# mateomarin/two_towers

Measured on AMD Instinct MI355X. Metric: training pairs/sec at global batch=8192, 1/2/4/8 GPUs; MRR@10 match, higher is better.
Workload: dtype bf16; 1 GPU; BASELINE configs[2]: EnhancedTwoTowerModel(300, 256), seq_len 64, batch 8192 per GPU, bf16, hard-negative mining k=5 + margin 0.2, dropout 0.1, Adam; global_batch=8192, seq_len=64, hidden=256, embedding_dim=300, parallelism=dp1, loss=hardneg_margin

## Files before the change

two_towers_amd/csrc/tt_api.h:

```cpp
#pragma once
#include <hip/hip_runtime.h>
#include <stdio.h>
#include <string.h>

#include "../../include/tt_hip.h"

namespace tt {
void set_error(const char* fmt, ...);

enum Opt {
  OPT_GRU_STEP,
  OPT_GRU_DEPTH,
  OPT_GRU_BWD_ROWS,
  OPT_GRU_BWD_BIG,
  OPT_GRU_BWD_STREAMS,
  OPT_GEMM_PERSIST,
  OPT_GEMM_A3,
  OPT_GEMM_REGSTAGE,
  OPT_GEMM_STREAM_OUT,
  OPT_HN_GEMM,
  OPT_GRU_BWD_PERSIST,
  OPT_GRU_FWD_STEP_ROWS,
  OPT_INFONCE_FLASH,
  OPT_HN_MAP,
  OPT_GEMM_SKEW,
  OPT_GEMM_PERSIST_MAXK,
  OPT_GRU_FWD_XC,
  OPT_GRU_XC_SKIP,
  OPT_GRU_XC_SPINS,
  OPT_GRU_BWD_SKEW,
  OPT_GRU_FWD_SKEW,
  OPT_GEMM_BRES,
  OPT_GRU_XC_COOP,
  OPT_GEMM_BUF,
  OPT_GEMM_ORDER,
  OPT_GRU_STEP_RING,
  OPT_GRU_FWD_XS,
  OPT_HN_SCAN_GEMM,
  OPT_GEMM_IEPI,
  OPT_BRES_ROWS,
  OPT_HN_SCAN_V,
  OPT_GEMM_W4,
  OPT_N
};
int opt(Opt o);
int tt_hn_scan_gemm(const void* q, long bq, const void* d, long nd, int h, long label_off, float* cm, long nch,
                    hipStream_t st);
}

#define TT_CHECK_ARG(cond, ...)            \
  do {                                     \
    if (!(cond)) {                         \
      tt::set_error(__VA_ARGS__);          \
      return TT_EINVAL;                    \
    }                                      \
  } while (0)

#define TT_CHECK_LAUNCH(what)                                                        \
  do {                                                                               \
    hipError_t e_ = hipGetLastError();                                               \
    if (e_ != hipSuccess) {                                                          \
      tt::set_error("%s: %s", what, hipGetErrorString(e_));                          \
      return (int)e_;                                                                \
    }                                                                                \
  } while (0)

#define TT_CHECK_HIP(expr)                                                           \
  do {                                                                               \
    hipError_t e_ = (expr);                                                          \
    if (e_ != hipSuccess) {                                                          \
      tt::set_error("%s: %s", #expr, hipGetErrorString(e_));                         \
      return (int)e_;                                                                \
    }                                                                                \
  } while (0)

#define TT_PROPAGATE(expr)     \
  do {                         \
    int rc_ = (expr);          \
    if (rc_ != 0) return rc_;  \
  } while (0)

static inline int tt_ceil_div(long a, long b) { return (int)((a + b - 1) / b); }
```

two_towers_amd/csrc/tt_gemm.hip:

```cpp
#include <float.h>
#include <stdarg.h>
#include <stdlib.h>

#include <atomic>
#include <type_traits>

#include "tt_api.h"
#include "tt_gemm_core.h"

namespace tt {
static thread_local char g_err[512];
void set_error(const char* fmt, ...) {
  va_list ap;
  va_start(ap, fmt);
  vsnprintf(g_err, sizeof(g_err), fmt, ap);
  va_end(ap);
}
}

namespace tt {
namespace {
struct OptDef {
  const char* name;
  const char* env;
  int dflt;
};
constexpr OptDef kOpts[OPT_N] = {
    {"gru_step", "TT_GRU_STEP", 0},               {"gru_depth", "TT_GRU_DEPTH", 4},
    {"gru_bwd_rows", "TT_GRU_BWD_ROWS", 0},     {"gru_bwd_big", "TT_GRU_BWD_BIG", 1},
    {"gru_bwd_streams", "TT_GRU_BWD_STREAMS", 2}, {"gemm_persist", "TT_GEMM_PERSIST", 1},
    {"gemm_a3", "TT_GEMM_A3", 1},                 {"gemm_regstage", "TT_GEMM_REGSTAGE", 0},
    {"gemm_stream_out", "TT_GEMM_STREAM_OUT", 1}, {"hn_gemm", "TT_HN_GEMM", 0},
    {"gru_bwd_persist", "TT_GRU_BWD_PERSIST", 1}, {"gru_fwd_step_rows", "TT_GRU_FWD_STEP_ROWS", 0},
    {"infonce_flash", "TT_INFONCE_FLASH", 1},     {"hn_map", "TT_HN_MAP", 2},
    {"gemm_skew", "TT_GEMM_SKEW", 0},             {"gemm_persist_maxk", "TT_GEMM_PERSIST_MAXK", 24},
    {"gru_fwd_xc", "TT_GRU_FWD_XC", 1},           {"gru_xc_skip", "TT_GRU_XC_SKIP", 0},
    {"gru_xc_spins", "TT_GRU_XC_SPINS", 22},      {"gru_bwd_skew", "TT_GRU_BWD_SKEW", 14},
    {"gru_fwd_skew", "TT_GRU_FWD_SKEW", 0},       {"gemm_bres", "TT_GEMM_BRES", 1},
    {"gru_xc_coop", "TT_GRU_XC_COOP", 0},         {"gemm_buf", "TT_GEMM_BUF", 1},
    {"gemm_order", "TT_GEMM_ORDER", 0},           {"gru_step_ring", "TT_GRU_STEP_RING", 4},
    {"gru_fwd_xs", "TT_GRU_FWD_XS", 1},           {"hn_scan_gemm", "TT_HN_SCAN_GEMM", 0},
    {"gemm_iepi", "TT_GEMM_IEPI", 1},             {"bres_rows", "TT_BRES_ROWS", 32},
    {"hn_scan_v", "TT_HN_SCAN_V", 5},             {"gemm_w4", "TT_GEMM_W4", 0},
};
struct OptTable {
  std::atomic<int> v[OPT_N];
  OptTable() {
    for (int i = 0; i < OPT_N; ++i) {
      const char* e = getenv(kOpts[i].env);
      v[i].store(e && *e ? atoi(e) : kOpts[i].dflt, std::memory_order_relaxed);
    }
  }
};
OptTable& opts() {
  static OptTable t;
  return t;
}
int find_opt(const char* name) {
  for (int i = 0; name && i < OPT_N; ++i)
    if (strcmp(name, kOpts[i].name) == 0) return i;
  return -1;
}
}
int opt(Opt o) { return opts().v[o].load(std::memory_order_relaxed); }
}

extern "C" const char* tt_version(void) { return "tt_hip 0.2.0 gfx950"; }
extern "C" const char* tt_last_error(void) { return tt::g_err; }
extern "C" int tt_set_option(const char* name, int value) {
  const int i = tt::find_opt(name);
  TT_CHECK_ARG(i >= 0, "tt_set_option: unknown option '%s'", name ? name : "(null)");
  tt::opts().v[i].store(value, std::memory_order_relaxed);
  return 0;
}
extern "C" int tt_get_option(const char* name, int* value) {
  const int i = tt::find_opt(name);
  TT_CHECK_ARG(i >= 0 && value, "tt_get_option: unknown option '%s'", name ? name : "(null)");
  *value = tt::opt((tt::Opt)i);
  return 0;
}

namespace {

struct GemmArgs {
  const void* a[4];
  const void* b[4];
  void* c[4];
  const float* bias[4];
  int bshift[4];
  const void* a_hi[4];
  int a_split;
  long lda, ldb, ldc;
  int M, N, K;
  int splits, kt_per_split;
  float alpha;
  int beta, relu, seq_t;
  uint32_t drop_seed, drop_thresh, drop_row0;
  float drop_inv_keep;
  long part_stride;
  int vec_ok;
  int force_regstage;
  int skew;
  int bias_vec_ok;
  int stream_out;
  int walk_g, walk_x;
  int nbatch;
  float* cm;
  long nch, label_off;
};

constexpr int BM = 128, BN = 128;

#ifndef TT_TAIL_SKIP
#define TT_TAIL_SKIP 1
#endif
using ttg::xcd_remap;
#ifndef PERSIST_IEPI
#define PERSIST_IEPI 1
#endif
#ifndef PERSIST_BAL
#define PERSIST_BAL 1
#endif
#ifndef TT_EPI_PAIR
#define TT_EPI_PAIR 1
#endif
#ifndef TT_GEMM_BAL
// ... 1383 lines not shown
```

two_towers_amd/csrc/tt_gru.hip:

```cpp
#include <algorithm>
#include <cstdlib>
#include <mutex>
#include <type_traits>

#include "tt_api.h"
#include "tt_gemm_core.h"

namespace {

struct FwdRec {
  const void* g; const void* whh; const float* bhn; void* y; void* x1; void* save; float* hs;
  int dir; uint32_t seed; int col0;
  uint32_t row0;
};
struct FwdArgs {
  FwdRec r[4];
  int B, T, H;
  long ldg, ldy;
  int s;
  uint32_t drop_thresh;
  float inv_keep;
#ifdef TT_DIAG
  int dbg;
#endif
// ... 242 lines not shown
        if (!last) ld8(cr_nxt + (long)b * H + j, cin);
        else if (R.dfinal) ld8(R.dfinal + (long)b * a.ldf + j, cin);
        else {
#pragma unroll
          for (int e = 0; e < 8; ++e) cin[e] = 0.f;
        }
        if (DY) ld8(DY + row * a.ldy + j, dy);
        else {
#pragma unroll
          for (int e = 0; e < 8; ++e) dy[e] = 0.f;
        }
        const T* sp = S + row * S4 + j;
        ld8(sp, ar);
        ld8(sp + H, az);
        ld8(sp + 2 * H, an);
        ld8(sp + 3 * H, gh);
        if (s > 0) ld8(Y + ((long)b * T_ + tp) * a.ldy + j, hp);
        else {
#pragma unroll
          for (int e = 0; e < 8; ++e) hp[e] = 0.f;
        }
        const float* Lc = L + rl * BLD + jg;
        float o_r[8], o_z[8], o_n[8], o_hn[8], cout[8];
#pragma unroll
        for (int e = 0; e < 8; ++e) {
          const float dht = Lc[e] + cin[e] + dy[e];
          float rg, omr, zg, omz, ng, sech2;
          tt_sigmoid_pair(ar[e], rg, omr);
          tt_sigmoid_pair(az[e], zg, omz);
          tt_tanh_sech2(an[e], ng, sech2);
          const float dnp = dht * omz * sech2;
          const float drp = dnp * gh[e] * rg * omr;
          const float dzp = dht * (hp[e] - ng) * zg * omz;
          o_r[e] = drp; o_z[e] = dzp; o_n[e] = dnp; o_hn[e] = dnp * rg;
          cout[e] = dht * zg;
          bsum[0][e] += drp; bsum[1][e] += dzp; bsum[2][e] += dnp; bsum[3][e] += dnp * rg;
        }
        st8(cr_cur + (long)b * H + j, cout);
        T* xw = DGXw + row * a.ldd + j;
        st8(xw, o_r);
        st8(xw + H, o_z);
        const int go = (int)((((long)(b - m0) * T_) * a.ldd + j + 2 * H) * (long)sizeof(T));
        st8_sc1(grs, go, o_n, (T*)nullptr);
        st8(DGHw + row * a.ldd + j, o_hn);
      }
    }
    __syncthreads();
  }
#pragma unroll
  for (int q = 0; q < 4; ++q)
#pragma unroll
    for (int e = 0; e < 8; ++e) {
      float v = bsum[q][e];
      v += __shfl_xor(v, 16, 64);
      v += __shfl_xor(v, 32, 64);
      bsum[q][e] = v;
    }
  float* red = L;
  if (lane < 16) {
#pragma unroll
    for (int q = 0; q < 4; ++q)
#pragma unroll
      for (int e = 0; e < 8; ++e) red[(wave * 4 + q) * 128 + lane * 8 + e] = bsum[q][e];
  }
  __syncthreads();
  if (tid < 128 && j0 + tid < H) {
    float* pb = R.dbias + (long)mt * (4L * H) + j0 + tid;
#pragma unroll
    for (int q = 0; q < 4; ++q)
      pb[q * H] += red[(0 * 4 + q) * 128 + tid] + red[(1 * 4 + q) * 128 + tid] + red[(2 * 4 + q) * 128 + tid] +
                   red[(3 * 4 + q) * 128 + tid];
  }
}

TT_DEV void unpack8(uint4 v, float (&f)[8]) {
  f[0] = __uint_as_float(v.x << 16); f[1] = __uint_as_float(v.x & 0xFFFF0000u);
  f[2] = __uint_as_float(v.y << 16); f[3] = __uint_as_float(v.y & 0xFFFF0000u);
  f[4] = __uint_as_float(v.z << 16); f[5] = __uint_as_float(v.z & 0xFFFF0000u);
  f[6] = __uint_as_float(v.w << 16); f[7] = __uint_as_float(v.w & 0xFFFF0000u);
}

#ifndef TT_BWD_BUF
#define TT_BWD_BUF 1
#endif
#ifndef TT_BWD_STAG
#define TT_BWD_STAG 0
#endif
#ifndef TT_BWD_NB
#define TT_BWD_NB 2
#endif
#ifndef TT_BWD_NT
#define TT_BWD_NT 3
#endif
#ifndef TT_BWD_PIPE
#define TT_BWD_PIPE 1
#endif
#ifndef TT_BWD_CREG
#define TT_BWD_CREG 1
#endif
#ifndef TT_BWD_OUT_NT
#define TT_BWD_OUT_NT 0
#endif
template <bool NT>
TT_DEV void st8_pol(bf16_t* p, const float (&f)[8]) {
  if constexpr (NT) {
    tt_u32x4 w;
#pragma unroll
    for (int i = 0; i < 4; ++i) w[i] = (uint32_t)f2bf(f[2 * i]) | ((uint32_t)f2bf(f[2 * i + 1]) << 16);
    __builtin_nontemporal_store(w, reinterpret_cast<tt_u32x4*>(p));
  } else {
    st8(p, f);
  }
}

__global__ __launch_bounds__(512) void gru_bwd_big(BwdArgs a) {
  using L8 = ttg::Loop8<bf16_t, false, true, false, false, false, TT_BWD_BUF != 0>;
  static_assert(L8::LDS_BYTES >= 128 * 256 * 4 && L8::LDS_BYTES >= 8 * 4 * 256 * 4, "staging fits the slots");
  __shared__ __attribute__((aligned(16))) char lds[L8::LDS_BYTES];
  const int H = a.H, T_ = a.T, s = a.s;
  const int ntj = (H + 255) / 256, ntm = (a.B + 255) / 256;
  const int id = ttg::xcd_remap(blockIdx.x, gridDim.x);
  const int rz = id / (ntm * ntj), rem = id - rz * ntm * ntj;
  const int mt = rem / ntj;
  const BwdRec R = a.r[rz];
  const int m0 = mt * 256, j0 = (rem % ntj) * 256;
  const int t = R.dir ? T_ - 1 - s : s;
  const int tn = R.dir ? t - 1 : t + 1;
  const int tp = R.dir ? t + 1 : t - 1;
  const bool last = (s == T_ - 1);
  const int wave = threadIdx.x >> 6, lane = threadIdx.x & 63, tid = threadIdx.x;
  const int wn = (wave & 3) * 64;

  f32x4 acc[8][4];
#pragma unroll
  for (int i = 0; i < 8; ++i)
#pragma unroll
    for (int j = 0; j < 4; ++j) acc[i][j] = f32x4{0.f, 0.f, 0.f, 0.f};
#ifdef TT_DIAG
  const int dbg = a.dbg;
#else
  constexpr int dbg = 0;
#endif
  if (!last && !(dbg & 1)) {
    const bf16_t* DGX = static_cast<const bf16_t*>(R.dgx);
    const bf16_t* DGH = static_cast<const bf16_t*>(R.dgh);
    ttg::KCSplit<bf16_t> la{DGX + (long)tn * a.ldd, DGH + (long)tn * a.ldd, (long)T_ * a.ldd, m0, a.B, 2 * H};
    ttg::KOPlain<bf16_t> lb{static_cast<const bf16_t*>(R.whh), H, j0, H - j0};
    L8::run(la, lb, 3 * H, 0, (3 * H + L8::KTE - 1) / L8::KTE, lds, acc);
  }

  float* L = reinterpret_cast<float*>(lds);
  const int cur = s & 1, nxt = cur ^ 1;
  const bf16_t* S = static_cast<const bf16_t*>(R.save);
  const bf16_t* Y = static_cast<const bf16_t*>(R.y);
  const bf16_t* DY = static_cast<const bf16_t*>(R.dy);
  bf16_t* DGXw = static_cast<bf16_t*>(R.dgx);
  bf16_t* DGHw = static_cast<bf16_t*>(R.dgh);
  bf16_t* cr_cur = static_cast<bf16_t*>(R.dh) + (long)cur * a.B * H;
  const bf16_t* cr_nxt = static_cast<const bf16_t*>(R.dh) + (long)nxt * a.B * H;
  const long S4 = 4L * H;
  const int jg = (tid & 31) * 8;
  const int j = j0 + jg;
  const __amdgpu_buffer_rsrc_t grs = tt_rsrc(DGXw + ((long)m0 * T_ + t) * a.ldd);
  const __amdgpu_buffer_rsrc_t rc = tt_rsrc_n(cr_nxt + (long)m0 * H, !last);
  const __amdgpu_buffer_rsrc_t rd = tt_rsrc_n(DY ? DY + ((long)m0 * T_ + t) * a.ldy : S, DY != nullptr);
  const __amdgpu_buffer_rsrc_t rsv = tt_rsrc_n(S + ((long)m0 * T_ + t) * S4, true);
  const __amdgpu_buffer_rsrc_t ry = tt_rsrc_n(s > 0 ? Y + ((long)m0 * T_ + tp) * a.ldy : S, s > 0);
  float bsum[4][8];
#pragma unroll
// ... 17 lines not shown
#pragma unroll
      for (int kk = 0; kk < NB; ++kk) {
        const int bl = (tid >> 5) + p * 64 + 16 * ((kb + kk) & 3) + 128 * ((kb + kk) >> 2);
        const bool ok = m0 + bl < a.B && !(dbg & 2);
        const uint32_t oc = ok ? (uint32_t)(bl * H + j) * 2u : 0x80000000u;
        const uint32_t oy = ok ? (uint32_t)(bl * T_ * (int)a.ldy + j) * 2u : 0x80000000u;
        const uint32_t os = ok ? (uint32_t)(bl * T_ * (int)S4 + j) * 2u : 0x80000000u;
        vin[kk][0] = ld16_buf(rc, oc, 0);
        vin[kk][1] = ld16_buf<(TT_BWD_NT & 2) ? 2 : 0>(rd, oy, 0);
#pragma unroll
        for (int q = 0; q < 4; ++q) vin[kk][2 + q] = ld16_buf<(TT_BWD_NT & 1) ? 2 : 0>(rsv, os, q * 2 * H);
        vin[kk][6] = ld16_buf<(TT_BWD_NT & 2) ? 2 : 0>(ry, oy, 0);
      }
#pragma unroll
      for (int kk = 0; kk < NB; ++kk) {
        const int rl = (tid >> 5) + 16 * (kb + kk);
        const int b = m0 + (rl >> 6) * 128 + p * 64 + (rl & 63);
        if (b >= a.B) continue;
        const long row = (long)b * T_ + t;
        float cin[8], dy[8], ar[8], az[8], an[8], gh[8], hp[8];
        unpack8(vin[kk][0], cin);
        unpack8(vin[kk][1], dy);
        unpack8(vin[kk][2], ar);
        unpack8(vin[kk][3], az);
        unpack8(vin[kk][4], an);
        unpack8(vin[kk][5], gh);
        unpack8(vin[kk][6], hp);
        if (last && R.dfinal) ld8(R.dfinal + (long)b * a.ldf + j, cin);
        const float* Lc = L + rl * 256 + jg;
        float o_r[8], o_z[8], o_n[8], o_hn[8], cout[8];
#pragma unroll
        for (int e = 0; e < 8; ++e) {
          const float dht = Lc[e] + cin[e] + dy[e];
          float rg, omr, zg, omz, ng, sech2;
          tt_sigmoid_pair(ar[e], rg, omr);
          tt_sigmoid_pair(az[e], zg, omz);
          tt_tanh_sech2(an[e], ng, sech2);
          const float dnp = dht * omz * sech2;
          const float drp = dnp * gh[e] * rg * omr;
          const float dzp = dht * (hp[e] - ng) * zg * omz;
          o_r[e] = drp; o_z[e] = dzp; o_n[e] = dnp; o_hn[e] = dnp * rg;
          cout[e] = dht * zg;
          bsum[0][e] += drp; bsum[1][e] += dzp; bsum[2][e] += dnp; bsum[3][e] += dnp * rg;
        }
        if (dbg & 4) {
          if (o_r[0] == 12345.f) L[0] = o_z[1] + o_n[2] + o_hn[3] + cout[4];
          continue;
        }
        st8(cr_cur + (long)b * H + j, cout);
        bf16_t* xw = DGXw + row * a.ldd + j;
        st8(xw, o_r);
        st8(xw + H, o_z);
        const int go = (int)((((long)(b - m0) * T_) * a.ldd + j + 2 * H) * 2L);
        st8_sc1(grs, go, o_n, (bf16_t*)nullptr);
        st8(DGHw + row * a.ldd + j, o_hn);
      }
    }
    __syncthreads();
  }
#pragma unroll
  for (int q = 0; q < 4; ++q)
#pragma unroll
    for (int e = 0; e < 8; ++e) bsum[q][e] += __shfl_xor(bsum[q][e], 32, 64);
  float* red = L;
  if (lane < 32) {
#pragma unroll
    for (int q = 0; q < 4; ++q)
#pragma unroll
      for (int e = 0; e < 8; ++e) red[(wave * 4 + q) * 256 + lane * 8 + e] = bsum[q][e];
  }
  __syncthreads();
  if (tid < 256 && j0 + tid < H) {
    float* pb = R.dbias + (long)(mt * 2) * (4L * H) + j0 + tid;
#pragma unroll
    for (int q = 0; q < 4; ++q) {
      float v = 0.f;
#pragma unroll
      for (int w = 0; w < 8; ++w) v += red[(w * 4 + q) * 256 + tid];
      pb[q * H] += v;
    }
  }
}

template <int H>
struct BwdRowsCfg {
  static constexpr int NP = H > 512 ? H / 512 : 1;
  static constexpr int HP = H / NP;
  static constexpr int NQ = HP / 128;
  static constexpr int SLOT = 8192 + NQ * 8192;
  static constexpr int NS = 4;
  static constexpr int LDS = NS * SLOT;
  static constexpr int P = SLOT / 1024 / 8;
  static constexpr int NCB = HP / 64;
  static constexpr int TPR = HP / 8;
  static constexpr int RPI = 512 / TPR;
  static constexpr int LDB = HP + 8;
  static_assert(SLOT % 8192 == 0 && 128 * LDB * 2 <= LDS && RPI * 4 * HP * 4 <= LDS, "ring layout");
};

TT_DEV uint4 frag_kc64(const char* img, int r0) {
  const int lane = threadIdx.x & 63;
  const int row = r0 + (lane & 15);
  return *reinterpret_cast<const uint4*>(img + row * 64 + (((lane >> 4) ^ ((row >> 1) & 3)) << 4));
}

template <int N, int P>
TT_DEV void wait_younger(int n) {
  if constexpr (N > 0) {
    if (n >= N) {
      asm volatile("s_waitcnt vmcnt(%0)" ::"n"(P * N) : "memory");
      return;
    }
    wait_younger<N - 1, P>(n);
  } else {
    asm volatile("s_waitcnt vmcnt(0)" ::: "memory");
  }
}

template <int H>
__global__ __launch_bounds__(512) void gru_bwd_rows(BwdArgs a) {
  using C = BwdRowsCfg<H>;
  __shared__ __attribute__((aligned(16))) char lds[C::LDS];
  const int T_ = a.T, ntm = (a.B + 127) / 128;
  const int id = ttg::xcd_remap(blockIdx.x, gridDim.x);
  const int rz = id / ntm, mt = id - rz * ntm;
  const BwdRec R = a.r[rz];
  const int m0 = mt * 128;
  const int tid = threadIdx.x, wave = tid >> 6, lane = tid & 63;
  const int wr = wave >> 2, wc = wave & 3;
  const bf16_t* DGX = static_cast<const bf16_t*>(R.dgx);
  const bf16_t* DGH = static_cast<const bf16_t*>(R.dgh);
  bf16_t* DGXw = static_cast<bf16_t*>(R.dgx);
  bf16_t* DGHw = static_cast<bf16_t*>(R.dgh);
  const bf16_t* S = static_cast<const bf16_t*>(R.save);
  const bf16_t* Y = static_cast<const bf16_t*>(R.y);
  const bf16_t* DY = static_cast<const bf16_t*>(R.dy);
  const bf16_t* W = static_cast<const bf16_t*>(R.whh);
  const uint32_t lbase = __builtin_amdgcn_readfirstlane(ttg::lds_addr_of(lds));
  constexpr int NK = 3 * H / 32;
  if (a.skew != 0) {
    const int ph = a.skew > 0 ? (int)((blockIdx.x >> 3) & 1) : (int)((blockIdx.x >> 3) & 3);
    const int n = ph * (a.skew > 0 ? a.skew : -a.skew);
    for (int i = 0; i < n; ++i) __builtin_amdgcn_s_sleep(127);
  }
  const long ldr = (long)T_ * a.ldd;
  int prow[C::P], pcol[C::P];
#pragma unroll
  for (int j = 0; j < C::P; ++j) {
    const int pc = wave + 8 * j, q = (pc & 7) * 64 + lane;
    if (pc < 8) {
      const int row = q >> 2;
      prow[j] = row;
      pcol[j] = ((q & 3) ^ ((row >> 1) & 3)) * 8;
    } else {
      const int sub = (pc - 8) >> 3, kl = q >> 4;
      prow[j] = -1;
      pcol[j] = kl * H + sub * 128 + (((q & 15) ^ (ttg::ko_v(kl) << 1)) * 8);
    }
  }
  const int jg = (tid % C::TPR) * 8, rsub = tid / C::TPR;
  float* L = reinterpret_cast<float*>(lds);
  float* part = R.dbias + (long)mt * (4L * H);
  const char* zp = reinterpret_cast<const char*>(ttg::g_tt_zero_page);
#ifdef TT_DIAG
  const int dbg = a.dbg;
#else
  constexpr int dbg = 0;
#endif

  constexpr bool CREG = TT_BWD_CREG != 0 && C::NP == 1;
  constexpr int NIT = 128 / C::RPI;
  static_assert(!CREG || 128 * C::LDB * 2 + C::RPI * C::HP * 4 <= C::LDS, "carry image + one bias row of partials");
  static_assert(!CREG || C::HP <= 512, "one bias column per thread");
  float bacc[4][8];
#pragma unroll
  for (int q = 0; q < 4; ++q)
#pragma unroll
    for (int e = 0; e < 8; ++e) bacc[q][e] = 0.f;
  for (int s = T_ - 1; s >= 0; --s) {
    const int t = R.dir ? T_ - 1 - s : s;
    const int tn = R.dir ? t - 1 : t + 1;
    const int tp = R.dir ? t + 1 : t - 1;
    const bool last = (s == T_ - 1);
    auto column_pass = [&](const int u0) {
    f32x4 acc[4][C::NCB];
#pragma unroll
    for (int i = 0; i < 4; ++i)
#pragma unroll
      for (int j = 0; j < C::NCB; ++j) acc[i][j] = f32x4{0.f, 0.f, 0.f, 0.f};
    if (CREG && !last) {
#pragma unroll
      for (int i = 0; i < 4; ++i)
#pragma unroll
        for (int jc = 0; jc < C::NCB; ++jc) {
          const uint2 w = *reinterpret_cast<const uint2*>(reinterpret_cast<const bf16_t*>(lds) +
                                                          (wr * 64 + 16 * i + (lane & 15)) * C::LDB + wc * (C::HP / 4) +
                                                          16 * jc + 4 * (lane >> 4));
          acc[i][jc] = f32x4{__uint_as_float(w.x << 16), __uint_as_float(w.x & 0xFFFF0000u),
                             __uint_as_float(w.y << 16), __uint_as_float(w.y & 0xFFFF0000u)};
        }
      __syncthreads();
    }
    if (!last && !(dbg & 1)) {
#if TT_BWD_BUF
      const long abytes = (long)(a.B - m0) * ldr * 2;
      const uint32_t anrec = (uint32_t)(abytes > 0xFFFFFFFFL ? 0xFFFFFFFFL : abytes);
      const ttg::tt_rsrc4 rsx = ttg::make_rsrc4(DGX + (long)tn * a.ldd + (long)m0 * ldr, anrec);
      const ttg::tt_rsrc4 rsh = ttg::make_rsrc4(DGH + (long)tn * a.ldd + (long)m0 * ldr - 2 * H, anrec);
      const ttg::tt_rsrc4 rsw = ttg::make_rsrc4(W + u0, 0xFFFFFFFFu);
      uint32_t voff[C::P];
#pragma unroll
      for (int j = 0; j < C::P; ++j)
        voff[j] = prow[j] >= 0 ? (uint32_t)(((long)prow[j] * ldr + pcol[j]) * 2) : (uint32_t)(pcol[j] * 2);
      auto issue = [&](int r) {
        const uint32_t img = lbase + (uint32_t)(r % C::NS) * C::SLOT;
        const int wv = __builtin_amdgcn_readfirstlane(threadIdx.x >> 6);
        const bool hi = r * 32 >= 2 * H;
#pragma unroll
        for (int j = 0; j < C::P; ++j) {
          const int pc = wv + 8 * j;
          if (pc < 8) ttg::dma16_buf(hi ? rsh : rsx, voff[j], (uint32_t)r * 64u, img + (uint32_t)pc * 1024u);
          else ttg::dma16_buf(rsw, voff[j], (uint32_t)r * (uint32_t)(64 * H), img + (uint32_t)pc * 1024u);
        }
      };
#else
      const char* as0[C::P];
      const char* as1[C::P];
#pragma unroll
      for (int j = 0; j < C::P; ++j) {
        const int b = m0 + (prow[j] < 0 ? 0 : prow[j]);
        const bool ok = prow[j] >= 0 && b < a.B;
        as0[j] = ok ? reinterpret_cast<const char*>(DGX + (long)tn * a.ldd + (long)b * ldr + pcol[j]) : zp;
        as1[j] = ok ? reinterpret_cast<const char*>(DGH + (long)tn * a.ldd + (long)b * ldr + pcol[j] - 2 * H) : zp;
      }
      auto issue = [&](int r) {
        const uint32_t img = lbase + (uint32_t)(r % C::NS) * C::SLOT;
        const int wv = __builtin_amdgcn_readfirstlane(threadIdx.x >> 6);
        const bool hi = r * 32 >= 2 * H;
#pragma unroll
        for (int j = 0; j < C::P; ++j) {
          const int pc = wv + 8 * j;
          const char* src;
          if (pc < 8) {
            src = hi ? as1[j] : as0[j];
            if (src != zp) src += (long)r * 64;
          } else {
            src = reinterpret_cast<const char*>(W + (long)r * 32 * H + u0 + pcol[j]);
          }
          ttg::dma16(src, img + (uint32_t)pc * 1024u);
        }
      };
#endif
      issue(0);
      issue(1);
      issue(2);
#if TT_BWD_STAG
      const bool late = wr == 1;
      wait_younger<C::NS - 2, C::P>(NK - 1);
      __builtin_amdgcn_s_barrier();
      if (late) __builtin_amdgcn_s_barrier();
#pragma unroll 1
      for (int r = 0; r < NK; ++r) {
        if (r > 0) __builtin_amdgcn_s_barrier();
        if (r + 3 < NK) issue(r + 3);
        const char* sl = lds + (r % C::NS) * C::SLOT;
        uint4 fa[4], fb[C::NCB];
#pragma unroll
        for (int i = 0; i < 4; ++i) fa[i] = frag_kc64(sl, wr * 64 + 16 * i);
        const char* ib = sl + 8192 + ((wc * (C::HP / 4)) >> 7) * 8192;
        const int cb = (wc * (C::HP / 4)) & 127;
#pragma unroll
        for (int j = 0; j < C::NCB; ++j) fb[j] = ttg::frag<bf16_t, true>(ib, cb + 16 * j, 0);
        __builtin_amdgcn_s_setprio(1);
#pragma unroll
        for (int j = 0; j < C::NCB / 2; ++j)
#pragma unroll
          for (int i = 0; i < 4; ++i) acc[i][j] = ttg::mma<bf16_t>(fb[j], fa[i], acc[i][j]);
        __builtin_amdgcn_s_setprio(0);
        asm volatile("s_waitcnt lgkmcnt(0)" ::: "memory");
        __builtin_amdgcn_sched_barrier(0);
        if (late) wait_younger<C::NS - 2, C::P>(NK - 2 - r);
        __builtin_amdgcn_s_barrier();
        __builtin_amdgcn_s_setprio(1);
#pragma unroll
        for (int j = C::NCB / 2; j < C::NCB; ++j)
#pragma unroll
          for (int i = 0; i < 4; ++i) acc[i][j] = ttg::mma<bf16_t>(fb[j], fa[i], acc[i][j]);
        __builtin_amdgcn_s_setprio(0);
        if (!late) wait_younger<C::NS - 2, C::P>(NK - 2 - r);
      }
      if (!late) __builtin_amdgcn_s_barrier();
#else
#pragma unroll 1
      for (int r = 0; r < NK; ++r) {
        wait_younger<C::NS - 2, C::P>(NK - 1 - r);
        __builtin_amdgcn_s_barrier();
        if (r + 3 < NK) issue(r + 3);
        const char* sl = lds + (r % C::NS) * C::SLOT;
        uint4 fa[4];
#pragma unroll
        for (int i = 0; i < 4; ++i) fa[i] = frag_kc64(sl, wr * 64 + 16 * i);
        const char* ib = sl + 8192 + ((wc * (C::HP / 4)) >> 7) * 8192;
        const int cb = (wc * (C::HP / 4)) & 127;
#pragma unroll
        for (int jp = 0; jp < C::NCB; jp += 2) {
          uint4 fb[2];
#pragma unroll
          for (int j = 0; j < 2; ++j) fb[j] = ttg::frag<bf16_t, true>(ib, cb + 16 * (jp + j), 0);
          __builtin_amdgcn_s_setprio(1);
#pragma unroll
          for (int i = 0; i < 4; ++i)
#pragma unroll
            for (int j = 0; j < 2; ++j)
              acc[i][jp + j] = ttg::mma<bf16_t>(fb[j], fa[i], acc[i][jp + j]);
          __builtin_amdgcn_s_setprio(0);
        }
      }
#endif
      __builtin_amdgcn_s_barrier();
    }
    const long trow = (long)m0 * T_ + t;
    const __amdgpu_buffer_rsrc_t rc =
        tt_rsrc_n(static_cast<const bf16_t*>(R.dh) + (long)((s + 1) & 1) * a.B * H + (long)m0 * H, !last);
    bf16_t* cr_cur = static_cast<bf16_t*>(R.dh) + (long)(s & 1) * a.B * H + (long)m0 * H;
    const __amdgpu_buffer_rsrc_t rd = tt_rsrc_n(DY ? DY + trow * a.ldy : S, DY != nullptr);
    const __amdgpu_buffer_rsrc_t rsv = tt_rsrc_n(S + trow * 4L * H, true);
    const __amdgpu_buffer_rsrc_t ry = tt_rsrc_n(s > 0 ? Y + ((long)m0 * T_ + tp) * a.ldy : S, s > 0);
    const __amdgpu_buffer_rsrc_t grs = tt_rsrc(DGXw + trow * a.ldd);
    uint32_t* L16 = reinterpret_cast<uint32_t*>(lds);
#pragma unroll
    for (int i = 0; i < 4; ++i)
#pragma unroll
      for (int jc = 0; jc < C::NCB; ++jc) {
        const uint32_t w0 = (uint32_t)f2bf(acc[i][jc][0]) | ((uint32_t)f2bf(acc[i][jc][1]) << 16);
        const uint32_t w1 = (uint32_t)f2bf(acc[i][jc][2]) | ((uint32_t)f2bf(acc[i][jc][3]) << 16);
        *reinterpret_cast<uint2*>(reinterpret_cast<bf16_t*>(lds) + (wr * 64 + 16 * i + (lane & 15)) * C::LDB +
                                  wc * (C::HP / 4) + 16 * jc + 4 * (lane >> 4)) = make_uint2(w0, w1);
      }
    __syncthreads();
    float bsum_own[4][8];
    auto& bsum = CREG ? bacc : bsum_own;
    if constexpr (!CREG) {
#pragma unroll
      for (int q = 0; q < 4; ++q)
#pragma unroll
        for (int e = 0; e < 8; ++e) bsum[q][e] = 0.f;
    }
    constexpr int NB = TT_BWD_NB;
    auto load_row = [&](const int k, uint4 (&v)[7]) {
      const int bl = rsub + C::RPI * k;
      const bool ok = k < NIT && m0 + bl < a.B && !(dbg & 2);
      const uint32_t oc = ok ? (uint32_t)(bl * H + u0 + jg) * 2u : 0x80000000u;
      const uint32_t oy = ok ? (uint32_t)(bl * T_ * (int)a.ldy + u0 + jg) * 2u : 0x80000000u;
      const uint32_t os = ok ? (uint32_t)(bl * T_ * 4 * H + u0 + jg) * 2u : 0x80000000u;
      v[0] = CREG ? make_uint4(0, 0, 0, 0) : ld16_buf(rc, oc, 0);
      v[1] = ld16_buf<(TT_BWD_NT & 2) ? 2 : 0>(rd, oy, 0);
#pragma unroll
      for (int q = 0; q < 4; ++q) v[2 + q] = ld16_buf<(TT_BWD_NT & 1) ? 2 : 0>(rsv, os, q * 2 * H);
      v[6] = ld16_buf<(TT_BWD_NT & 2) ? 2 : 0>(ry, oy, 0);
    };
    auto finish_row = [&](const int k, const uint4 (&v)[7]) {
      const int bl = rsub + C::RPI * k;
      const int b = m0 + bl;
      if (b >= a.B) return;
      float cin[8], dy[8], ar[8], az[8], an[8], gh[8], hp[8], gm[8];
      unpack8(v[0], cin);
      unpack8(v[1], dy);
      unpack8(v[2], ar);
      unpack8(v[3], az);
      unpack8(v[4], an);
      unpack8(v[5], gh);
      unpack8(v[6], hp);
      unpack8(*reinterpret_cast<const uint4*>(L16 + ((bl * C::LDB + jg) >> 1)), gm);
      if (last && R.dfinal) {
        const float* pf = R.dfinal + (long)b * a.ldf + u0 + jg;
        tt_u32x4 d0, d1;
        asm volatile("global_load_dwordx4 %0, %2, off\n\tglobal_load_dwordx4 %1, %2, off offset:16\n\ts_waitcnt vmcnt(0)"
                     : "=&v"(d0), "=&v"(d1)
                     : "v"(pf)
                     : "memory");
#pragma unroll
        for (int e = 0; e < 4; ++e) {
          cin[e] = __uint_as_float(d0[e]);
          cin[4 + e] = __uint_as_float(d1[e]);
        }
      }
      float o_r[8], o_z[8], o_n[8], o_hn[8], cout[8];
#pragma unroll
      for (int e = 0; e < 8; ++e) {
        const float dht = gm[e] + cin[e] + dy[e];
        float rg, omr, zg, omz, ng, sech2;
        tt_sigmoid_pair(ar[e], rg, omr);
        tt_sigmoid_pair(az[e], zg, omz);
        tt_tanh_sech2(an[e], ng, sech2);
        const float dnp = dht * omz * sech2;
        const float drp = dnp * gh[e] * rg * omr;
        const float dzp = dht * (hp[e] - ng) * zg * omz;
        o_r[e] = drp; o_z[e] = dzp; o_n[e] = dnp; o_hn[e] = dnp * rg;
        cout[e] = dht * zg;
        bsum[0][e] += drp; bsum[1][e] += dzp; bsum[2][e] += dnp; bsum[3][e] += dnp * rg;
      }
// ... 1325 lines not shown
  const int esz = dtype == TT_DT_BF16 ? 2 : 4;
  TT_CHECK_ARG(H % 8 == 0 && (ldy * esz) % 16 == 0, "tt_gru_fwd: H=%d (multiple of 8)/ldy=%ld misaligned", H, ldy);
  TT_CHECK_ARG(drop_p >= 0.f && drop_p < 1.f, "tt_gru_fwd: drop_p");
  TT_CHECK_ARG(tt_ceil_div(B, 128) <= 65535, "tt_gru_fwd: B too large");
  TT_CHECK_ARG(128L * T * std::max({4L * H, ldy, ldg}) * esz < (1L << 31), "tt_gru_fwd: tile byte offsets exceed 2 GiB");
  FwdArgs a{};
  for (int i = 0; i < nrec; ++i) {
    const tt_gru_fwd_rec& r = recs[i];
    TT_CHECK_ARG(r.g && r.whh && r.bhn && r.y && r.save && r.hstate, "tt_gru_fwd: null pointer in rec %d", i);
    a.r[i] = FwdRec{r.g, r.whh, r.bhn, r.y, r.x1, r.save, r.hstate, r.dir, r.drop_seed, r.drop_col0, r.drop_row0};
  }
  a.B = B; a.T = T; a.H = H; a.ldg = ldg; a.ldy = ldy;
  a.drop_thresh = drop_p > 0.f ? (uint32_t)(drop_p * 16777216.0f + 0.5f) : 0u;
  a.inv_keep = drop_p > 0.f ? 1.0f / (1.0f - drop_p) : 1.0f;
#ifdef TT_DIAG
  if (const char* e = getenv("TT_GRU_DBG")) a.dbg = atoi(e);
#endif
  hipStream_t st = (hipStream_t)stream;
  if (dtype == TT_DT_BF16) {
    bool used = false;
    TT_PROPAGATE(gru_fwd_xc_launch(a, nrec, B, T, H, ldg, ldy, ws, ws_bytes, st, &used));
    if (used) return 0;
  }
  if (gru_fwd_persistent(dtype, H)) return launch_fwd_seq(a, nrec, B, H, st);
  return launch_fwd_steps(dtype, a, nrec, B, T, H, ldg, ldy, st);
}

extern "C" long tt_gru_infer_scratch_size(int dtype, int B, int T, int H, int final_only) {
  if ((dtype != TT_DT_F32 && dtype != TT_DT_BF16) || B <= 0 || T <= 0 || H <= 0) return 0;
  if (gru_fwd_persistent(dtype, H)) return 0;
  const long esz = dtype == TT_DT_BF16 ? 2 : 4;
  return 2L * B * H * 4 + (final_only ? 2L * B * H * esz : 0);
}

extern "C" int tt_gru_fwd_infer(int dtype, const tt_gru_infer_rec* recs, int nrec, int B, int T, int H, long ldg,
                                long ldy, long ldf, void* ws, long ws_bytes, void* stream) {
  TT_CHECK_ARG(dtype == TT_DT_F32 || dtype == TT_DT_BF16, "tt_gru_fwd_infer: bad dtype");
  TT_CHECK_ARG(nrec >= 1 && nrec <= 4, "tt_gru_fwd_infer: nrec %d", nrec);
  TT_CHECK_ARG(B > 0 && T > 0 && H > 0, "tt_gru_fwd_infer: bad shape");
  TT_CHECK_ARG(ws_bytes >= 0 && (ws != nullptr || ws_bytes == 0), "tt_gru_fwd_infer: ws / ws_bytes");
  const int esz = dtype == TT_DT_BF16 ? 2 : 4;
  TT_CHECK_ARG(H % 8 == 0 && (ldy * esz) % 16 == 0, "tt_gru_fwd_infer: H=%d (multiple of 8)/ldy=%ld misaligned", H, ldy);
  TT_CHECK_ARG(tt_ceil_div(B, 128) <= 65535, "tt_gru_fwd_infer: B too large");
  TT_CHECK_ARG(128L * T * std::max({4L * H, ldy, ldg}) * esz < (1L << 31),
               "tt_gru_fwd_infer: tile byte offsets exceed 2 GiB");
  const bool has_y = recs[0].y != nullptr, has_f = recs[0].hfinal != nullptr;
  TT_CHECK_ARG(has_y || has_f, "tt_gru_fwd_infer: neither y nor hfinal given");
  TT_CHECK_ARG(!has_f || (ldf >= H && (ldf * esz) % 16 == 0 && 256L * ldf * esz < (1L << 31)),
               "tt_gru_fwd_infer: ldf=%ld misaligned or below H", ldf);
  const bool persistent = gru_fwd_persistent(dtype, H);
  const long state = 2L * B * H * 4;
  InfArgs a{};
  for (int i = 0; i < nrec; ++i) {
    const tt_gru_infer_rec& r = recs[i];
    TT_CHECK_ARG(r.g && r.whh && r.bhn, "tt_gru_fwd_infer: null pointer in rec %d", i);
    TT_CHECK_ARG((r.y != nullptr) == has_y && (r.hfinal != nullptr) == has_f,
                 "tt_gru_fwd_infer: rec %d disagrees with rec 0 on y / hfinal", i);
    TT_CHECK_ARG(persistent || (r.scratch && ((uintptr_t)r.scratch & 15) == 0),
                 "tt_gru_fwd_infer: rec %d needs 16-byte aligned scratch (tt_gru_infer_scratch_size)", i);
    a.r[i] = FwdRec{r.g, r.whh, r.bhn, r.y, nullptr, nullptr, static_cast<float*>(r.scratch), r.dir, 0u, 0, 0u};
    for (int k = nrec; k < 4; ++k) a.hfin[k] = a.himg[k] = nullptr;
    a.hfin[i] = r.hfinal;
    a.himg[i] = r.scratch && !has_y ? static_cast<char*>(r.scratch) + state : nullptr;
  }
  a.B = B; a.T = T; a.H = H; a.ldg = ldg; a.ldy = ldy; a.ldf = ldf;
  a.inv_keep = 1.0f;
  hipStream_t st = (hipStream_t)stream;
  if (dtype == TT_DT_BF16) {
    bool used = false;
    TT_PROPAGATE(gru_fwd_xc_launch(a, nrec, B, T, H, ldg, ldy, ws, ws_bytes, st, &used));
    if (used) return 0;
  }
  if (persistent) return launch_fwd_seq(a, nrec, B, H, st);
  return launch_fwd_steps(dtype, a, nrec, B, T, H, ldg, ldy, st);
}

template <typename T, int BMR>
static void launch_bwd_step(int ring, dim3 grid, hipStream_t st, const BwdArgs& a) {
  if (ring >= 4) hipLaunchKernelGGL((gru_bwd_step<T, BMR, 4>), grid, dim3(256), 0, st, a);
  else if (ring == 3) hipLaunchKernelGGL((gru_bwd_step<T, BMR, 3>), grid, dim3(256), 0, st, a);
  else hipLaunchKernelGGL((gru_bwd_step<T, BMR>), grid, dim3(256), 0, st, a);
}

extern "C" int tt_gru_bwd(int dtype, const tt_gru_bwd_rec* recs, int nrec, int B, int T, int H, long ldy,
                          long ldd, long ldf, void* stream) {
  TT_CHECK_ARG(dtype == TT_DT_F32 || dtype == TT_DT_BF16, "tt_gru_bwd: bad dtype");
  TT_CHECK_ARG(nrec >= 1 && nrec <= 4, "tt_gru_bwd: nrec %d", nrec);
  TT_CHECK_ARG(B > 0 && T > 0 && H > 0, "tt_gru_bwd: bad shape");
  const int esz = dtype == TT_DT_BF16 ? 2 : 4;
  TT_CHECK_ARG(H % 8 == 0 && (ldd * esz) % 16 == 0, "tt_gru_bwd: H=%d (multiple of 8)/ldd=%ld misaligned", H, ldd);
  TT_CHECK_ARG(256L * T * std::max({ldd, ldy, 4L * H}) * esz < (1L << 31), "tt_gru_bwd: tile byte offsets exceed 2 GiB");
  hipStream_t st = (hipStream_t)stream;
  BwdArgs a{};
  for (int i = 0; i < nrec; ++i) {
    const tt_gru_bwd_rec& r = recs[i];
    TT_CHECK_ARG(r.save && r.y && r.whh && r.dgx && r.dgh && r.dhstate && r.dbias_part,
                 "tt_gru_bwd: null pointer in rec %d", i);
    a.r[i] = BwdRec{r.save, r.y, r.dy, r.dfinal, r.whh, r.dgx, r.dgh, r.dhstate, r.dbias_part, r.dir};
    TT_CHECK_HIP(hipMemsetAsync(r.dbias_part, 0, sizeof(float) * 4L * H * tt_gru_bias_rows(B), st));
  }
  a.B = B; a.T = T; a.H = H; a.ldy = ldy; a.ldd = ldd; a.ldf = ldf;
  a.skew = tt::opt(tt::OPT_GRU_BWD_SKEW);
#ifdef TT_DIAG
  if (const char* e = getenv("TT_GRU_DBG")) a.dbg = atoi(e);
#endif
  const int bmr = bwd_rows(B, H, nrec);
  if (gru_bwd_persistent(dtype, H)) {
    TT_CHECK_ARG(128L * T * std::max({ldd, ldy, 4L * H}) * esz < (1L << 31), "tt_gru_bwd: tile offsets exceed 2 GiB");
    const dim3 grid(tt_ceil_div(B, 128) * nrec);
    if (H == 1024) hipLaunchKernelGGL(gru_bwd_rows<1024>, grid, dim3(512), 0, st, a);
    else if (H == 512) hipLaunchKernelGGL(gru_bwd_rows<512>, grid, dim3(512), 0, st, a);
    else hipLaunchKernelGGL(gru_bwd_rows<256>, grid, dim3(512), 0, st, a);
    TT_CHECK_LAUNCH("gru_bwd_rows");
    return 0;
  }
  if (dtype == TT_DT_BF16 && H % 256 == 0 && bmr == 128 && tt::opt(tt::OPT_GRU_BWD_BIG) != 0) {
    const dim3 grid((H / 256) * tt_ceil_div(B, 256) * nrec);
    for (int s = T - 1; s >= 0; --s) {
      a.s = s;
      hipLaunchKernelGGL(gru_bwd_big, grid, dim3(512), 0, st, a);
      TT_CHECK_LAUNCH("gru_bwd_big");
    }
    return 0;
  }
  const int ngrp = (nrec >= 2 && tt::opt(tt::OPT_GRU_BWD_STREAMS) != 1) ? 2 : 1;
  BwdArgs ga[2] = {a, a};
  int gn[2] = {nrec, 0};
  if (ngrp == 2) {
    gn[0] = nrec / 2;
    gn[1] = nrec - gn[0];
    for (int i = 0; i < gn[1]; ++i) ga[1].r[i] = a.r[gn[0] + i];
  }
  hipStream_t gs[2] = {st, st};
  SideStream* side = nullptr;
  if (ngrp == 2) {
    TT_PROPAGATE(side_stream(&side));
    gs[1] = side->s;
    TT_CHECK_HIP(hipEventRecord(side->fork, st));
    TT_CHECK_HIP(hipStreamWaitEvent(side->s, side->fork, 0));
  }
  XcDev* xd = nullptr;
  TT_PROPAGATE(xc_device(&xd));
  long wgs = 0;
  for (int g = 0; g < ngrp; ++g) wgs += (long)tt_ceil_div(H, 128) * tt_ceil_div(B, bmr) * gn[g];
  const int ring = wgs <= xd->cus ? tt::opt(tt::OPT_GRU_STEP_RING) : 2;
  for (int s = T - 1; s >= 0; --s) {
    for (int g = 0; g < ngrp; ++g) {
      ga[g].s = s;
      const dim3 grid(tt_ceil_div(H, 128) * tt_ceil_div(B, bmr) * gn[g]);
      if (dtype == TT_DT_BF16) {
        if (bmr == 64) launch_bwd_step<bf16_t, 64>(ring, grid, gs[g], ga[g]);
        else launch_bwd_step<bf16_t, 128>(ring, grid, gs[g], ga[g]);
      } else {
        if (bmr == 64) launch_bwd_step<float, 64>(ring, grid, gs[g], ga[g]);
        else launch_bwd_step<float, 128>(ring, grid, gs[g], ga[g]);
      }
      TT_CHECK_LAUNCH("gru_bwd_step");
    }
  }
  if (ngrp == 2) {
    TT_CHECK_HIP(hipEventRecord(side->join, side->s));
    TT_CHECK_HIP(hipStreamWaitEvent(st, side->join, 0));
  }
  return 0;
}
```

Before: 152,300 pairs/s.

## Add split activation/weight LDS rings with wave specialization to GRU backward rows kernel

```diff
diff --git a/two_towers_amd/csrc/tt_api.h b/two_towers_amd/csrc/tt_api.h
--- a/two_towers_amd/csrc/tt_api.h
+++ b/two_towers_amd/csrc/tt_api.h
@@ -41,6 +41,7 @@
   OPT_BRES_ROWS,
   OPT_HN_SCAN_V,
   OPT_GEMM_W4,
+  OPT_GRU_BWD_RING,
   OPT_N
 };
 int opt(Opt o);
diff --git a/two_towers_amd/csrc/tt_gemm.hip b/two_towers_amd/csrc/tt_gemm.hip
--- a/two_towers_amd/csrc/tt_gemm.hip
+++ b/two_towers_amd/csrc/tt_gemm.hip
@@ -42,6 +42,7 @@
     {"gru_fwd_xs", "TT_GRU_FWD_XS", 1},           {"hn_scan_gemm", "TT_HN_SCAN_GEMM", 0},
     {"gemm_iepi", "TT_GEMM_IEPI", 1},             {"bres_rows", "TT_BRES_ROWS", 32},
     {"hn_scan_v", "TT_HN_SCAN_V", 5},             {"gemm_w4", "TT_GEMM_W4", 0},
+    {"gru_bwd_ring", "TT_GRU_BWD_RING", 0},
 };
 struct OptTable {
   std::atomic<int> v[OPT_N];
diff --git a/two_towers_amd/csrc/tt_gru.hip b/two_towers_amd/csrc/tt_gru.hip
--- a/two_towers_amd/csrc/tt_gru.hip
+++ b/two_towers_amd/csrc/tt_gru.hip
@@ -348,9 +348,6 @@
 
 #ifndef TT_BWD_BUF
 #define TT_BWD_BUF 1
-#endif
-#ifndef TT_BWD_STAG
-#define TT_BWD_STAG 0
 #endif
 #ifndef TT_BWD_NB
 #define TT_BWD_NB 2
@@ -534,20 +531,29 @@
   }
 }
 
-template <int H>
+template <int H, int RING = 0>
 struct BwdRowsCfg {
   static constexpr int NP = H > 512 ? H / 512 : 1;
   static constexpr int HP = H / NP;
   static constexpr int NQ = HP / 128;
-  static constexpr int SLOT = 8192 + NQ * 8192;
-  static constexpr int NS = 4;
-  static constexpr int LDS = NS * SLOT;
-  static constexpr int P = SLOT / 1024 / 8;
+  static constexpr int WS = NQ * 8192;
+  static constexpr int SLOT = 8192 + WS;
+  static constexpr bool SPLIT = RING != 0;
+  static constexpr int NSW = RING == 1 ? 1 + 65536 / WS : 4;
+  static constexpr int NSA = RING == 1 ? 8 : 4;
+  static constexpr int WOFF = RING == 1 ? 0 : 8192, WSTEP = RING == 1 ? WS : SLOT;
+  static constexpr int AOFF = RING == 1 ? NSW * WS : 0, ASTEP = RING == 1 ? 8192 : SLOT;
+  static constexpr int LDS = RING == 1 ? NSW * WS + NSA * 8192 : 4 * SLOT;
+  static constexpr int NWV = SPLIT ? 4 : 8;
+  static constexpr int PA = 8 / NWV;
+  static constexpr int PW = NQ * 8 / NWV;
   static constexpr int NCB = HP / 64;
   static constexpr int TPR = HP / 8;
   static constexpr int RPI = 512 / TPR;
   static constexpr int LDB = HP + 8;
-  static_assert(SLOT % 8192 == 0 && 128 * LDB * 2 <= LDS && RPI * 4 * HP * 4 <= LDS, "ring layout");
+  static_assert(RING >= 0 && RING <= 2 && NSW >= 3 && NSA >= 3, "a ring keeps at least two K-tiles in flight");
+  static_assert(LDS <= 160 * 1024 && 128 * LDB * 2 <= LDS && RPI * 4 * HP * 4 <= LDS, "ring layout");
+  static_assert((NSW - 2) * (SPLIT ? PW : PA + PW) < 64 && (NSA - 2) * PA < 64, "counted waits fit vmcnt");
 };
 
 TT_DEV uint4 frag_kc64(const char* img, int r0) {
@@ -569,9 +575,9 @@
   }
 }
 
-template <int H>
+template <int H, int RING>
 __global__ __launch_bounds__(512) void gru_bwd_rows(BwdArgs a) {
-  using C = BwdRowsCfg<H>;
+  using C = BwdRowsCfg<H, RING>;
   __shared__ __attribute__((aligned(16))) char lds[C::LDS];
   const int T_ = a.T, ntm = (a.B + 127) / 128;
   const int id = ttg::xcd_remap(blockIdx.x, gridDim.x);
@@ -595,30 +601,39 @@
     const int n = ph * (a.skew > 0 ? a.skew : -a.skew);
     for (int i = 0; i < n; ++i) __builtin_amdgcn_s_sleep(127);
   }
+  const int wv = __builtin_amdgcn_readfirstlane(threadIdx.x >> 6);
+  const bool wv_a = !C::SPLIT || wv >= 4, wv_w = !C::SPLIT || wv < 4;
+  const int wvr = C::SPLIT ? (wv & 3) : wv;
+  constexpr int JW = 8 / C::NWV;
+  uint32_t va[C::PA], vw[JW];
   const long ldr = (long)T_ * a.ldd;
-  int prow[C::P], pcol[C::P];
-#pragma unroll
-  for (int j = 0; j < C::P; ++j) {
-    const int pc = wave + 8 * j, q = (pc & 7) * 64 + lane;
-    if (pc < 8) {
-      const int row = q >> 2;
-      prow[j] = row;
-      pcol[j] = ((q & 3) ^ ((row >> 1) & 3)) * 8;
-    } else {
-      const int sub = (pc - 8) >> 3, kl = q >> 4;
-      prow[j] = -1;
-      pcol[j] = kl * H + sub * 128 + (((q & 15) ^ (ttg::ko_v(kl) << 1)) * 8);
-    }
+#pragma unroll
+  for (int j = 0; j < C::PA; ++j) {
+    const int q = (wvr + C::NWV * j) * 64 + lane, row = q >> 2;
+    va[j] = (uint32_t)(((long)row * ldr + ((q & 3) ^ ((row >> 1) & 3)) * 8) * 2);
+  }
+#pragma unroll
+  for (int j = 0; j < JW; ++j) {
+    const int q = (wvr + C::NWV * j) * 64 + lane, kl = q >> 4;
+    vw[j] = (uint32_t)((kl * H + (((q & 15) ^ (ttg::ko_v(kl) << 1)) * 8)) * 2);
   }
   const int jg = (tid % C::TPR) * 8, rsub = tid / C::TPR;
   float* L = reinterpret_cast<float*>(lds);
   float* part = R.dbias + (long)mt * (4L * H);
-  const char* zp = reinterpret_cast<const char*>(ttg::g_tt_zero_page);
 #ifdef TT_DIAG
   const int dbg = a.dbg;
 #else
   constexpr int dbg = 0;
 #endif
+  const uint32_t keep_a = ((uint32_t)(dbg >> 3) & 1u) - 1u, keep_w = ((uint32_t)(dbg >> 4) & 1u) - 1u;
+  auto uni = [](uint32_t v) {
+#ifdef TT_DIAG
+    v = (uint32_t)__builtin_amdgcn_readfirstlane(v);
+#endif
+    return v;
+  };
+#pragma unroll
+  for (int j = 0; j < C::PA; ++j) va[j] = (va[j] & keep_a) | ((uint32_t)lane * 16u & ~keep_a);
 
   constexpr bool CREG = TT_BWD_CREG != 0 && C::NP == 1;
   constexpr int NIT = 128 / C::RPI;
@@ -654,105 +669,52 @@
       __syncthreads();
     }
     if (!last && !(dbg & 1)) {
-#if TT_BWD_BUF
       const long abytes = (long)(a.B - m0) * ldr * 2;
       const uint32_t anrec = (uint32_t)(abytes > 0xFFFFFFFFL ? 0xFFFFFFFFL : abytes);
-      const ttg::tt_rsrc4 rsx = ttg::make_rsrc4(DGX + (long)tn * a.ldd + (long)m0 * ldr, anrec);
-      const ttg::tt_rsrc4 rsh = ttg::make_rsrc4(DGH + (long)tn * a.ldd + (long)m0 * ldr - 2 * H, anrec);
+      const bf16_t* ax = DGX + (long)tn * a.ldd + (long)m0 * ldr;
+      const bf16_t* ah = DGH + (long)tn * a.ldd + (long)m0 * ldr - 2 * H;
+      if (dbg & 8) ax = ah = reinterpret_cast<const bf16_t*>(ttg::g_tt_zero_page);
+      const ttg::tt_rsrc4 rsx = ttg::make_rsrc4(ax, (dbg & 8) ? 1024u : anrec);
+      const ttg::tt_rsrc4 rsh = ttg::make_rsrc4(ah, (dbg & 8) ? 1024u : anrec);
       const ttg::tt_rsrc4 rsw = ttg::make_rsrc4(W + u0, 0xFFFFFFFFu);
-      uint32_t voff[C::P];
-#pragma unroll
-      for (int j = 0; j < C::P; ++j)
-        voff[j] = prow[j] >= 0 ? (uint32_t)(((long)prow[j] * ldr + pcol[j]) * 2) : (uint32_t)(pcol[j] * 2);
-      auto issue = [&](int r) {
-        const uint32_t img = lbase + (uint32_t)(r % C::NS) * C::SLOT;
-        const int wv = __builtin_amdgcn_readfirstlane(threadIdx.x >> 6);
-        const bool hi = r * 32 >= 2 * H;
-#pragma unroll
-        for (int j = 0; j < C::P; ++j) {
-          const int pc = wv + 8 * j;
-          if (pc < 8) ttg::dma16_buf(hi ? rsh : rsx, voff[j], (uint32_t)r * 64u, img + (uint32_t)pc * 1024u);
-          else ttg::dma16_buf(rsw, voff[j], (uint32_t)r * (uint32_t)(64 * H), img + (uint32_t)pc * 1024u);
-        }
+      auto issue_a = [&](int r) {
+        if (!wv_a) return;
+        const uint32_t img = lbase + (uint32_t)(C::AOFF + (r % C::NSA) * C::ASTEP);
+        const uint32_t so = uni(((uint32_t)r * 64u) & keep_a);
+#pragma unroll
+        for (int j = 0; j < C::PA; ++j)
+          ttg::dma16_buf(r * 32 >= 2 * H ? rsh : rsx, va[j], so, img + (uint32_t)(wvr + C::NWV * j) * 1024u);
       };
-#else
-      const char* as0[C::P];
-      const char* as1[C::P];
-#pragma unroll
-      for (int j = 0; j < C::P; ++j) {
-        const int b = m0 + (prow[j] < 0 ? 0 : prow[j]);
-        const bool ok = prow[j] >= 0 && b < a.B;
-        as0[j] = ok ? reinterpret_cast<const char*>(DGX + (long)tn * a.ldd + (long)b * ldr + pcol[j]) : zp;
-        as1[j] = ok ? reinterpret_cast<const char*>(DGH + (long)tn * a.ldd + (long)b * ldr + pcol[j] - 2 * H) : zp;
-      }
-      auto issue = [&](int r) {
-        const uint32_t img = lbase + (uint32_t)(r % C::NS) * C::SLOT;
-        const int wv = __builtin_amdgcn_readfirstlane(threadIdx.x >> 6);
-        const bool hi = r * 32 >= 2 * H;
-#pragma unroll
-        for (int j = 0; j < C::P; ++j) {
-          const int pc = wv + 8 * j;
-          const char* src;
-          if (pc < 8) {
-            src = hi ? as1[j] : as0[j];
-            if (src != zp) src += (long)r * 64;
-          } else {
-            src = reinterpret_cast<const char*>(W + (long)r * 32 * H + u0 + pcol[j]);
-          }
-          ttg::dma16(src, img + (uint32_t)pc * 1024u);
-        }
+      auto issue_w = [&](int r) {
+        if (!wv_w) return;
+        const uint32_t img = lbase + (uint32_t)(C::WOFF + (r % C::NSW) * C::WSTEP);
+        const uint32_t so = uni(((uint32_t)r * (uint32_t)(64 * H)) & keep_w);
+#pragma unroll
+        for (int j = 0; j < C::PW; ++j)
+          ttg::dma16_buf(rsw, vw[j % JW], so + (uint32_t)(j / JW) * 256u, img + (uint32_t)(wvr + C::NWV * j) * 1024u);
       };
-#endif
-      issue(0);
-      issue(1);
-      issue(2);
-#if TT_BWD_STAG
-      const bool late = wr == 1;
-      wait_younger<C::NS - 2, C::P>(NK - 1);
-      __builtin_amdgcn_s_barrier();
-      if (late) __builtin_amdgcn_s_barrier();
+      auto landed = [&](int r) {
+        if constexpr (!C::SPLIT) wait_younger<C::NSW - 2, C::PA + C::PW>(NK - 1 - r);
+        else if (wv_w) wait_younger<C::NSW - 2, C::PW>(NK - 1 - r);
+        else wait_younger<C::NSA - 2, C::PA>(NK - 1 - r);
+      };
+      static_assert(NK >= C::NSA && NK >= C::NSW, "the step prologue fills both rings");
+#pragma unroll
+      for (int r = 0; r < (C::NSA > C::NSW ? C::NSA : C::NSW) - 1; ++r) {
+        if (r < C::NSA - 1) issue_a(r);
+        if (r < C::NSW - 1) issue_w(r);
+      }
 #pragma unroll 1
       for (int r = 0; r < NK; ++r) {
-        if (r > 0) __builtin_amdgcn_s_barrier();
-        if (r + 3 < NK) issue(r + 3);
-        const char* sl = lds + (r % C::NS) * C::SLOT;
-        uint4 fa[4], fb[C::NCB];
-#pragma unroll
-        for (int i = 0; i < 4; ++i) fa[i] = frag_kc64(sl, wr * 64 + 16 * i);
-        const char* ib = sl + 8192 + ((wc * (C::HP / 4)) >> 7) * 8192;
-        const int cb = (wc * (C::HP / 4)) & 127;
-#pragma unroll
-        for (int j = 0; j < C::NCB; ++j) fb[j] = ttg::frag<bf16_t, true>(ib, cb + 16 * j, 0);
-        __builtin_amdgcn_s_setprio(1);
-#pragma unroll
-        for (int j = 0; j < C::NCB / 2; ++j)
-#pragma unroll
-          for (int i = 0; i < 4; ++i) acc[i][j] = ttg::mma<bf16_t>(fb[j], fa[i], acc[i][j]);
-        __builtin_amdgcn_s_setprio(0);
-        asm volatile("s_waitcnt lgkmcnt(0)" ::: "memory");
-        __builtin_amdgcn_sched_barrier(0);
-        if (late) wait_younger<C::NS - 2, C::P>(NK - 2 - r);
+        landed(r);
         __builtin_amdgcn_s_barrier();
-        __builtin_amdgcn_s_setprio(1);
-#pragma unroll
-        for (int j = C::NCB / 2; j < C::NCB; ++j)
-#pragma unroll
-          for (int i = 0; i < 4; ++i) acc[i][j] = ttg::mma<bf16_t>(fb[j], fa[i], acc[i][j]);
-        __builtin_amdgcn_s_setprio(0);
-        if (!late) wait_younger<C::NS - 2, C::P>(NK - 2 - r);
-      }
-      if (!late) __builtin_amdgcn_s_barrier();
-#else
-#pragma unroll 1
-      for (int r = 0; r < NK; ++r) {
-        wait_younger<C::NS - 2, C::P>(NK - 1 - r);
-        __builtin_amdgcn_s_barrier();
-        if (r + 3 < NK) issue(r + 3);
-        const char* sl = lds + (r % C::NS) * C::SLOT;
+        if (r + C::NSA - 1 < NK) issue_a(r + C::NSA - 1);
+        if (r + C::NSW - 1 < NK) issue_w(r + C::NSW - 1);
+        const char* sa = lds + C::AOFF + (r % C::NSA) * C::ASTEP;
         uint4 fa[4];
 #pragma unroll
-        for (int i = 0; i < 4; ++i) fa[i] = frag_kc64(sl, wr * 64 + 16 * i);
-        const char* ib = sl + 8192 + ((wc * (C::HP / 4)) >> 7) * 8192;
+        for (int i = 0; i < 4; ++i) fa[i] = frag_kc64(sa, wr * 64 + 16 * i);
+        const char* ib = lds + C::WOFF + (r % C::NSW) * C::WSTEP + ((wc * (C::HP / 4)) >> 7) * 8192;
         const int cb = (wc * (C::HP / 4)) & 127;
 #pragma unroll
         for (int jp = 0; jp < C::NCB; jp += 2) {
@@ -768,7 +730,6 @@
           __builtin_amdgcn_s_setprio(0);
         }
       }
-#endif
       __builtin_amdgcn_s_barrier();
     }
     const long trow = (long)m0 * T_ + t;
@@ -2260,6 +2221,13 @@
   else hipLaunchKernelGGL((gru_bwd_step<T, BMR>), grid, dim3(256), 0, st, a);
 }
 
+template <int H>
+static void launch_bwd_rows(int ring, dim3 grid, hipStream_t st, const BwdArgs& a) {
+  if (ring == 1) hipLaunchKernelGGL((gru_bwd_rows<H, 1>), grid, dim3(512), 0, st, a);
+  else if (ring == 2) hipLaunchKernelGGL((gru_bwd_rows<H, 2>), grid, dim3(512), 0, st, a);
+  else hipLaunchKernelGGL((gru_bwd_rows<H, 0>), grid, dim3(512), 0, st, a);
+}
+
 extern "C" int tt_gru_bwd(int dtype, const tt_gru_bwd_rec* recs, int nrec, int B, int T, int H, long ldy,
                           long ldd, long ldf, void* stream) {
   TT_CHECK_ARG(dtype == TT_DT_F32 || dtype == TT_DT_BF16, "tt_gru_bwd: bad dtype");
@@ -2286,9 +2254,11 @@
   if (gru_bwd_persistent(dtype, H)) {
     TT_CHECK_ARG(128L * T * std::max({ldd, ldy, 4L * H}) * esz < (1L << 31), "tt_gru_bwd: tile offsets exceed 2 GiB");
     const dim3 grid(tt_ceil_div(B, 128) * nrec);
-    if (H == 1024) hipLaunchKernelGGL(gru_bwd_rows<1024>, grid, dim3(512), 0, st, a);
-    else if (H == 512) hipLaunchKernelGGL(gru_bwd_rows<512>, grid, dim3(512), 0, st, a);
-    else hipLaunchKernelGGL(gru_bwd_rows<256>, grid, dim3(512), 0, st, a);
+    const int ring = tt::opt(tt::OPT_GRU_BWD_RING);
+    TT_CHECK_ARG(ring >= 0 && ring <= 2, "tt_gru_bwd: option gru_bwd_ring %d", ring);
+    if (H == 1024) launch_bwd_rows<1024>(ring, grid, st, a);
+    else if (H == 512) launch_bwd_rows<512>(ring, grid, st, a);
+    else launch_bwd_rows<256>(ring, grid, st, a);
     TT_CHECK_LAUNCH("gru_bwd_rows");
     return 0;
   }
```

Result: no change. 152,800 pairs/s (median of 6 runs) (+0.3%).
